# sauloal/pykmer

Hardware: AMD Instinct MI355X
Metric: bp/s k-mer counted (k=15, 1 GPU) (higher is better)
Workload: dtype u8

## Files before the change

### pykmer_amd/csrc/kmer_part.hip

```cpp
#include <cstddef>
#include "part_common.h"

namespace pk {

__global__ __launch_bounds__(1024) void k_sample2(const uint32_t *__restrict__ in, const uint32_t *__restrict__ bucket_base,
                                                  const uint32_t *__restrict__ bucket_end, PartPlan pl, uint32_t stride2,
                                                  uint32_t *__restrict__ tally, uint32_t *__restrict__ sampled_n,
                                                  const uint32_t *__restrict__ flags) {
    __shared__ uint32_t h[512];
    __shared__ uint32_t n_seen;
    if (flags[0]) return;
    const uint32_t b = blockIdx.x, lo = bucket_base[b], hi = bucket_end[b];
    if (threadIdx.x < 512) h[threadIdx.x] = 0;
    if (threadIdx.x == 0) n_seen = 0;
    __syncthreads();
    const uint32_t n_grp = (hi - lo + 255u) / 256u, n_sgrp = (n_grp + stride2 - 1u) / stride2;
    const uint32_t mask = pl.B2 - 1u, shift = pl.fb_bits, w = threadIdx.x >> 6, lane = threadIdx.x & 63u;
    uint32_t mine = 0;
    for (uint32_t s0 = 0; s0 < n_sgrp; s0 += 8u * 16u) {
        uint4 v[8];
        uint32_t n_ok[8];
#pragma unroll
        for (int u = 0; u < 8; u++) {
            const uint32_t sg = s0 + (uint32_t)u * 16u + w;
            const uint64_t i = (uint64_t)lo + (uint64_t)sg * stride2 * 256u + lane * 4u;
            n_ok[u] = (sg < n_sgrp && i < hi) ? (uint32_t)min((uint64_t)4, (uint64_t)hi - i) : 0u;
            v[u] = n_ok[u] ? *reinterpret_cast<const uint4 *>(in + i) : make_uint4(0, 0, 0, 0);
        }
#pragma unroll
        for (int u = 0; u < 8; u++) {
            const uint32_t r4[4] = {v[u].x, v[u].y, v[u].z, v[u].w};
#pragma unroll
            for (uint32_t e = 0; e < 4; e++)
                if (e < n_ok[u]) { atomicAdd(&h[(r4[e] >> shift) & mask], 1u); mine++; }
        }
    }
    for (int d = 32; d; d >>= 1) mine += __shfl_down(mine, d, 64);
    if ((threadIdx.x & 63) == 0 && mine) atomicAdd(&n_seen, mine);
    __syncthreads();
    if (threadIdx.x < pl.B2) tally[(uint64_t)b * pl.B2 + threadIdx.x] = h[threadIdx.x];
    if (threadIdx.x == 0) sampled_n[b] = n_seen;
}
__global__ __launch_bounds__(1024) void k_rooms2(const uint32_t *__restrict__ tally, const uint32_t *__restrict__ sampled_n,
                                                 const uint32_t *__restrict__ bucket_base, const uint32_t *__restrict__ bucket_end, PartPlan pl,
                                                 uint32_t stride2, uint32_t n_final, uint32_t *__restrict__ final_start,
                                                 uint32_t *__restrict__ cap2_end, uint32_t *__restrict__ block_tot, const uint32_t *__restrict__ flags) {
    __shared__ uint32_t wsum[16];
    if (flags[0]) return;
    const uint32_t i = blockIdx.x * 1024u + threadIdx.x;
    uint32_t room = 0;
    if (i < n_final) {
        const uint32_t b = i >> pl.b2, hcount = tally[i];
        if (stride2 == 1u) room = hcount;
        else {
            const uint32_t seen = sampled_n[b], n_b = bucket_end[b] - bucket_base[b];
            const unsigned long long est = seen ? (unsigned long long)((double)hcount * ((double)n_b / (double)seen)) + 1ull : 0ull;
            room = (uint32_t)(est + est / 4 + 4096u);
        }
        room = (room + 7u) & ~7u;
    }
    uint32_t inc = room;
    const int lane = threadIdx.x & 63, w = threadIdx.x >> 6;
#pragma unroll
    for (int d = 1; d < 64; d <<= 1) { const uint32_t o = __shfl_up(inc, d, 64); if (lane >= d) inc += o; }
    if (lane == 63) wsum[w] = inc;
    __syncthreads();
    uint32_t pre = 0, total = 0;
    for (int j = 0; j < 16; j++) { if (j < w) pre += wsum[j]; total += wsum[j]; }
    if (i < n_final) { final_start[i] = pre + inc - room; cap2_end[i] = room; }
    if (threadIdx.x == 0) block_tot[blockIdx.x] = total;
}
__global__ __launch_bounds__(1024) void k_bases2(uint32_t n_blocks, uint32_t n_final, PartPlan pl, uint32_t *__restrict__ block_tot,
                                                 uint32_t *__restrict__ final_start, uint32_t *__restrict__ flags) {
    __shared__ uint32_t wsum[16];
    if (flags[0]) return;
    const uint32_t v = threadIdx.x < n_blocks ? block_tot[threadIdx.x] : 0u;
    uint32_t inc = v;
    const int lane = threadIdx.x & 63, w = threadIdx.x >> 6;
#pragma unroll
    for (int d = 1; d < 64; d <<= 1) { const uint32_t o = __shfl_up(inc, d, 64); if (lane >= d) inc += o; }
    if (lane == 63) wsum[w] = inc;
    __syncthreads();
    uint32_t pre = 0, total = 0;
    for (int j = 0; j < 16; j++) { if (j < w) pre += wsum[j]; total += wsum[j]; }
    if (threadIdx.x < n_blocks) block_tot[threadIdx.x] = pre + inc - v;
    __shared__ unsigned long long total64;
    if (threadIdx.x == 0) total64 = 0ull;
    __syncthreads();
    unsigned long long mine = v;
    for (int d = 32; d; d >>= 1) mine += __shfl_down(mine, d, 64);
    if (lane == 0 && mine) atomicAdd(&total64, mine);
    __syncthreads();
    if (threadIdx.x == 0) {
        final_start[n_final] = total;
        if (total64 > pl.capacity2) flags[0] = 1u;
    }
}
__global__ __launch_bounds__(1024) void k_starts2(uint32_t n_final, const uint32_t *__restrict__ block_base, uint32_t *__restrict__ final_start,
                                                  uint32_t *__restrict__ cursor2, uint32_t *__restrict__ cap2_end, const uint32_t *__restrict__ flags) {
    if (flags[0]) return;
    const uint32_t i = blockIdx.x * 1024u + threadIdx.x;
    if (i >= n_final) return;
    const uint32_t a = block_base[blockIdx.x] + final_start[i];
    final_start[i] = a; cursor2[i] = a; cap2_end[i] = a + cap2_end[i];
}

template <int NT, int PER, bool REC24 = false>
__global__ __launch_bounds__(NT, 4) void k_scatter2(const uint32_t *__restrict__ in, const uint32_t *__restrict__ wg2_start,
                                                   const uint32_t *__restrict__ bucket_base, const uint32_t *__restrict__ bucket_end, PartPlan pl,
                                                   void *__restrict__ out, uint32_t *__restrict__ cursor, const uint32_t *__restrict__ cap_end,
                                                   uint32_t dump, uint32_t *__restrict__ flags) {
    extern __shared__ __attribute__((aligned(16))) uint8_t smem[];
    ScatterLds &L = *reinterpret_cast<ScatterLds *>(smem);
    if (flags[0]) return;
    const uint32_t B = pl.B2, shift = pl.fb_bits;
    const uint32_t low_mask = (1u << shift) - 1u;
    for (uint32_t i = threadIdx.x; i < 512; i += NT) { L.hist[i] = 0; L.run[i] = 0; }
    __syncthreads();
    typedef uint32_t Quad __attribute__((ext_vector_type(4)));
    typedef uint32_t Pair __attribute__((ext_vector_type(2)));
    const uint16_t *in_lo = reinterpret_cast<const uint16_t *>(in);
    const uint8_t *in_hi = reinterpret_cast<const uint8_t *>(in) + level1_hi_plane_offset(pl.capacity1);
    auto item = [&](uint32_t b, uint32_t lo, uint32_t hi) {
        auto fetch = [&](uint32_t win, Quad (&v)[PER / 4]) {
            const uint32_t v_hi = min(hi, win + (uint32_t)TILE);
#pragma unroll
            for (int j = 0; j < PER / 4; j++) {
                const uint32_t i = win + (threadIdx.x + j * NT) * 4u;
                v[j] = Quad{0u, 0u, 0u, 0u};
                if (i < v_hi) {
                    if (REC24) {
                        const Pair l = *reinterpret_cast<const Pair *>(in_lo + i);
                        v[j] = Quad{l.x, l.y, *reinterpret_cast<const uint32_t *>(in_hi + i), 0u};
                    } else v[j] = *reinterpret_cast<const Quad *>(in + i);
                }
            }
        };
        Quad nxt[PER / 4];
        auto settle = [&]() {
            __builtin_amdgcn_s_waitcnt(0x0F70);
#pragma unroll
            for (int j = 0; j < PER / 4; j++) asm volatile("" : "+v"(nxt[j]));
        };
        fetch(lo & ~3u, nxt);
        settle();
        for (uint32_t win = lo & ~3u; win < hi; win += TILE) {
            const uint32_t v_lo = max(lo, win), v_hi = min(hi, win + (uint32_t)TILE);
            const uint32_t n_tile = v_hi - v_lo;
            uint32_t r[PER];
#pragma unroll
            for (int j = 0; j < PER / 4; j++) {
                if (REC24) {
                    r[j * 4] = __builtin_amdgcn_perm(nxt[j].z, nxt[j].x, 0x0c040100u);
                    r[j * 4 + 1] = __builtin_amdgcn_perm(nxt[j].z, nxt[j].x, 0x0c050302u);
                    r[j * 4 + 2] = __builtin_amdgcn_perm(nxt[j].z, nxt[j].y, 0x0c060100u);
                    r[j * 4 + 3] = __builtin_amdgcn_perm(nxt[j].z, nxt[j].y, 0x0c070302u);
                } else { r[j * 4] = nxt[j].x; r[j * 4 + 1] = nxt[j].y; r[j * 4 + 2] = nxt[j].z; r[j * 4 + 3] = nxt[j].w; }
            }
            const bool full = v_lo == win && n_tile == (uint32_t)TILE;
            uint32_t okm = 0;
            if (!full) {
#pragma unroll
                for (int j = 0; j < PER / 4; j++) {
                    const uint32_t i = win + (threadIdx.x + j * NT) * 4u;
#pragma unroll
                    for (int e = 0; e < 4; e++) okm |= (i + e >= v_lo && i + e < v_hi) ? (1u << (j * 4 + e)) : 0u;
                }
            }
            if (win + TILE < hi) fetch(win + TILE, nxt);
            uint32_t *cl = cursor + (uint64_t)b * B;
            const uint32_t *ce = cap_end + (uint64_t)b * B;
            if (full) scatter_tile<uint32_t, false, NT, PER, 512, true, 8, REC24>(L, r, 0u, n_tile, shift, B, low_mask, true, out, settle, cl, ce, dump, flags);
            else scatter_tile<uint32_t, false, NT, PER, 512, false, 8, REC24>(L, r, okm, n_tile, shift, B, low_mask, true, out, settle, cl, ce, dump, flags);
        }
    };
    const uint32_t *pos = wg2_start;
    const uint32_t per = pl.B1 >> 3;
    const uint32_t o_lo = (blockIdx.x & 7u) * per, o_hi = o_lo + per, first = blockIdx.x >> 3, step = gridDim.x >> 3;
    const uint32_t w_end = pos[o_hi];
    for (uint32_t w = pos[o_lo] + first; w < w_end; w += step) {
        uint32_t a = o_lo, z = o_hi;
        while (z - a > 1) { const uint32_t m = (a + z) >> 1; if (pos[m] <= w) a = m; else z = m; }
        const uint32_t b = (a % per) * 8u + a / per;
        const uint64_t s = (uint64_t)bucket_base[b] + (uint64_t)(w - pos[a]) * pl.R2;
        const uint64_t e = min(s + pl.R2, (uint64_t)bucket_end[b]);
        item(b, (uint32_t)s, (uint32_t)e);
    }
}

constexpr uint32_t K6_PIECE = 65024;
constexpr int K6_BYTES_LDS = 65536 + 1024 + 128;

__device__ __forceinline__ int wave_sum_i32(int v) {
    v += __builtin_amdgcn_update_dpp(0, v, 0x128, 0xf, 0xf, false);
    v += __builtin_amdgcn_update_dpp(0, v, 0x124, 0xf, 0xf, false);
    v += __builtin_amdgcn_update_dpp(0, v, 0x122, 0xf, 0xf, false);
    v += __builtin_amdgcn_update_dpp(0, v, 0x121, 0xf, 0xf, false);
    return __builtin_amdgcn_readlane(v, 0) + __builtin_amdgcn_readlane(v, 16) + __builtin_amdgcn_readlane(v, 32) +
           __builtin_amdgcn_readlane(v, 48);
}

typedef unsigned short U16x2 __attribute__((ext_vector_type(2)));
__device__ __forceinline__ uint32_t clamp255_pair(uint32_t x) {
    const U16x2 lim = {255, 255};
    return __builtin_bit_cast(uint32_t, __builtin_elementwise_min(__builtin_bit_cast(U16x2, x), lim));
}
__device__ __forceinline__ uint32_t pack_low_bytes(uint32_t x0, uint32_t x1) {
    return __builtin_amdgcn_perm(x1, x0, 0x06040200u);
}

struct SliceTally {
    int d1 = 0, d2 = 0;
    __device__ __forceinline__ void add_dword(int *dh, uint32_t x, int sign) {
        uint32_t p0 = x & 0x01010101u, p1 = (x >> 1) & 0x01010101u;
        uint32_t rest = p0 & p1;
        const uint32_t high = x & 0xfcfcfcfcu;
        if (high) {
            const uint32_t big = (((high & 0x7f7f7f7fu) + 0x7f7f7f7fu) | high) & 0x80808080u;
            const uint32_t keep = ~(big >> 7);
            p0 &= keep; p1 &= keep;
            rest = (p0 & p1) | (big >> 7);
        }
        const int n1 = (int)__builtin_popcount(p0 & ~p1), n2 = (int)__builtin_popcount(p1 & ~p0);
        d1 += sign * n1; d2 += sign * n2;
        while (rest) {
            const int bit = __ffs(rest) - 1;
            atomicAdd(&dh[(x >> bit) & 0xffu], sign);
            rest &= rest - 1u;
        }
    }
};

template <int T, bool LEAN, bool NOREC = false>
__device__ __forceinline__ void bucket_count_body(const uint16_t *__restrict__ recs, const uint32_t *__restrict__ final_start,
                                                  const uint32_t *__restrict__ final_end, uint32_t fb_bits, uint32_t split_bits,
                                                  uint8_t *__restrict__ table8, uint32_t fresh, unsigned long long *__restrict__ hist_rep, uint8_t *smem,
                                                  int *dh, uint32_t wg) {
    uint32_t *cnt = reinterpret_cast<uint32_t *>(smem);
    const uint32_t fb = wg >> split_bits, part = wg & ((1u << split_bits) - 1u);
    const uint32_t start = final_start[fb], end = final_end ? final_end[fb] : final_start[fb + 1];
    const uint32_t part_bits = fb_bits - split_bits;
    const uint32_t n_addr = 1u << part_bits;
    uint8_t *slice = table8 + ((uint64_t)fb << fb_bits) + (uint64_t)part * n_addr;
    if (start == end) {
        if (fresh) {
            if (n_addr >= 16) for (uint32_t g = threadIdx.x; g < n_addr / 16; g += T) reinterpret_cast<uint4 *>(slice)[g] = make_uint4(0, 0, 0, 0);
            else for (uint32_t a = threadIdx.x; a < n_addr; a += T) slice[a] = 0;
        }
        return;
    }
    const uint32_t base = start & ~7u;
    const uint32_t i_first = base + threadIdx.x * 8;
    uint4 v_first = make_uint4(0, 0, 0, 0);
    if (i_first < min(base + K6_PIECE, end)) v_first = *reinterpret_cast<const uint4 *>(recs + i_first);
    const bool by_rec = NOREC ? false : (((end - start) >> split_bits) < n_addr / 4 || n_addr < 16);
    SliceTally tally;
    for (uint32_t i = threadIdx.x; i < 256; i += T) dh[i] = 0;
    if (fresh) {
        if (n_addr >= 8) for (uint32_t g = threadIdx.x; g < n_addr / 8; g += T) reinterpret_cast<uint4 *>(cnt)[g] = make_uint4(0, 0, 0, 0);
        else for (uint32_t a = threadIdx.x; a < max(n_addr / 2, 1u); a += T) cnt[a] = 0u;
    } else if (n_addr >= 16) {
        if (!by_rec) __syncthreads();
        for (uint32_t g = threadIdx.x; g < n_addr / 16; g += T) {
            uint4 v = reinterpret_cast<const uint4 *>(slice)[g];
            uint32_t w[4] = {v.x, v.y, v.z, v.w};
            if (!by_rec) {
#pragma unroll
                for (int q = 0; q < 4; q++) tally.add_dword(dh, w[q], -1);
            }
#pragma unroll
            for (int q = 0; q < 8; q++)
                cnt[g * 8 + q] = __builtin_amdgcn_perm(0u, w[q >> 1], (q & 1) ? 0x0c030c02u : 0x0c010c00u);
        }
    } else {
        for (uint32_t a = threadIdx.x; a < n_addr / 2; a += T) cnt[a] = slice[2 * a] | ((uint32_t)slice[2 * a + 1] << 16);
    }
    __syncthreads();
    auto bump = [&](uint32_t a, uint32_t n) {
        const uint32_t sh = 16u * (a & 1u);
        if (!by_rec) { atomicAdd(&cnt[a >> 1], n << sh); return; }
        int &d1 = tally.d1, &d2 = tally.d2;
        const uint32_t c = (atomicAdd(&cnt[a >> 1], n << sh) >> sh) & 0xffffu;
        const uint32_t oc = c > 255u ? 255u : c, nc = c + n > 255u ? 255u : c + n;
        if (oc == nc) return;
        if (nc == 1u) d1++;
        else if (nc == 2u && oc == 1u) { d2++; d1--; }
        else {
            atomicAdd(&dh[nc], 1);
            if (oc) atomicAdd(&dh[oc], -1);
        }
    };
    auto count8 = [&](const uint4 &v, uint32_t i) {
        const uint32_t w[4] = {v.x, v.y, v.z, v.w};
        if (LEAN && !by_rec) {
            const bool interior = i >= start && i + 8u <= end;
            uint8_t *cb = reinterpret_cast<uint8_t *>(cnt);
#pragma unroll
            for (int q = 0; q < 8; q++) {
                const uint32_t x = w[q >> 1];
                const uint32_t off = (q & 1) ? ((x >> 15) & 0x1fffcu) : ((x << 1) & 0x1fffcu);
                const uint32_t low = (q & 1) ? ((x >> 16) & 1u) : (x & 1u);
                uint32_t val = low * 0xffffu + 1u;
                if (!interior) val = (i + q >= start && i + q < end) ? val : 0u;
                __hip_atomic_fetch_add(reinterpret_cast<uint32_t *>(cb + off), val, __ATOMIC_RELAXED, __HIP_MEMORY_SCOPE_WORKGROUP);
            }
            return;
        }
        uint32_t pa = 0, pn = 0;
#pragma unroll
        for (int q = 0; q < 8; q++) {
            const uint32_t idx = i + q;
            const uint32_t full = (w[q >> 1] >> (16 * (q & 1))) & 0xffffu;
            const bool in = idx >= start && idx < end && (full >> part_bits) == part;
            const uint32_t a = full & (n_addr - 1u);
            if (in && pn && a == pa) pn++;
            else {
                if (pn) bump(pa, pn);
                pa = a; pn = in ? 1u : 0u;
            }
        }
        if (pn) bump(pa, pn);
    };
    auto count8_sparse = [&](const uint4 &v, uint32_t i) {
        const uint32_t w[4] = {v.x, v.y, v.z, v.w};
        uint32_t old[8];
        bool in[8];
        const bool interior = i >= start && i + 8u <= end;
#pragma unroll
        for (int q = 0; q < 8; q++) {
            const uint32_t idx = i + q;
            const uint32_t full = (w[q >> 1] >> (16 * (q & 1))) & 0xffffu;
            in[q] = (interior || (idx >= start && idx < end)) && (full >> part_bits) == part;
            const uint32_t a = full & (n_addr - 1u), sh = 16u * (a & 1u);
            old[q] = (atomicAdd(&cnt[a >> 1], in[q] ? (1u << sh) : 0u) >> sh) & 0xffffu;
        }
#pragma unroll
        for (int q = 0; q < 8; q++) {
            const uint32_t c = old[q];
            if (!in[q] || c >= 255u) continue;
            if (c == 0u) tally.d1++;
            else if (c == 1u) { tally.d2++; tally.d1--; }
            else { atomicAdd(&dh[c + 1u], 1); atomicAdd(&dh[c], -1); }
        }
    };
    constexpr int NIT = (K6_PIECE + T * 8 - 1) / (T * 8);
    if (end - base <= (uint32_t)T * 8u) {
        if (i_first < end) { if (by_rec) count8_sparse(v_first, i_first); else count8(v_first, i_first); }
        __syncthreads();
    } else {
        for (uint32_t p0 = base; p0 < end; p0 += K6_PIECE) {
            const uint32_t p1 = min(p0 + K6_PIECE, end);
            uint4 v[NIT];
#pragma unroll
            for (int it = 0; it < NIT; it++) {
                const uint32_t i = p0 + (threadIdx.x + it * T) * 8;
                v[it] = make_uint4(0, 0, 0, 0);
                if (i < p1) v[it] = (it == 0 && p0 == base) ? v_first : *reinterpret_cast<const uint4 *>(recs + i);
            }
#pragma unroll
            for (int it = 0; it < NIT; it++) {
                const uint32_t i = p0 + (threadIdx.x + it * T) * 8;
                if (i < p1) count8(v[it], i);
            }
            __syncthreads();
            if (p1 < end) {
                for (uint32_t a = threadIdx.x; a < max(n_addr / 2, 1u); a += T) {
                    cnt[a] = clamp255_pair(cnt[a]);
                }
                __syncthreads();
            }
        }
    }
    if (n_addr >= 16) {
        for (uint32_t g = threadIdx.x; g < n_addr / 16; g += T) {
            const uint4 c0 = reinterpret_cast<const uint4 *>(cnt)[g * 2], c1 = reinterpret_cast<const uint4 *>(cnt)[g * 2 + 1];
            const uint32_t o[4] = {pack_low_bytes(clamp255_pair(c0.x), clamp255_pair(c0.y)), pack_low_bytes(clamp255_pair(c0.z), clamp255_pair(c0.w)),
                                   pack_low_bytes(clamp255_pair(c1.x), clamp255_pair(c1.y)), pack_low_bytes(clamp255_pair(c1.z), clamp255_pair(c1.w))};
            if (!by_rec) {
#pragma unroll
                for (int q = 0; q < 4; q++) tally.add_dword(dh, o[q], 1);
            }
            reinterpret_cast<uint4 *>(slice)[g] = make_uint4(o[0], o[1], o[2], o[3]);
        }
    } else {
        for (uint32_t a = threadIdx.x; a < n_addr / 2; a += T) {
            uint32_t x = cnt[a], lo = x & 0xffffu, hi = x >> 16;
            slice[2 * a] = (uint8_t)(lo > 255u ? 255u : lo);
            slice[2 * a + 1] = (uint8_t)(hi > 255u ? 255u : hi);
        }
    }
    const int d1 = wave_sum_i32(tally.d1), d2 = wave_sum_i32(tally.d2);
    if ((threadIdx.x & 63) == 0) {
        if (d1) atomicAdd(&dh[1], d1);
        if (d2) atomicAdd(&dh[2], d2);
    }
    __syncthreads();
    for (uint32_t i = threadIdx.x; i < 256; i += T) {
        const int v = dh[i];
        if (v) atomicAdd(&hist_rep[(uint64_t)(blockIdx.x % HIST_REPLICAS) * 256 + i], (unsigned long long)(long long)v);
    }
}

template <int T>
__global__ __launch_bounds__(T) void k_bucket_count(const uint16_t *__restrict__ recs, const uint32_t *__restrict__ final_start,
                                                    const uint32_t *__restrict__ final_end, uint32_t fb_bits, uint32_t split_bits,
                                                    uint8_t *__restrict__ table8, uint32_t fresh, unsigned long long *__restrict__ hist_rep,
                                                    const uint32_t *__restrict__ flags) {
    extern __shared__ __attribute__((aligned(16))) uint8_t smem[];
    __shared__ int dh[256];
    if (flags[0]) return;
    bucket_count_body<T, true>(recs, final_start, final_end, fb_bits, split_bits, table8, fresh, hist_rep, smem, dh, blockIdx.x);
}
template <int T, bool FRESH>
__global__ __launch_bounds__(T) __attribute__((amdgpu_waves_per_eu(8, 8)))
void k_bucket_count_half_lean(const uint16_t *__restrict__ recs, const uint32_t *__restrict__ final_start, const uint32_t *__restrict__ final_end,
                              uint32_t fb_bits, uint32_t split_bits, uint8_t *__restrict__ table8, uint32_t fresh, unsigned long long *__restrict__ hist_rep,
                              const uint32_t *__restrict__ flags) {
    extern __shared__ __attribute__((aligned(16))) uint8_t smem[];
    __shared__ int dh[256];
    if (flags[0]) return;
    bucket_count_body<T, true, true>(recs, final_start, final_end, 15u, 0u, table8, FRESH ? 1u : 0u, hist_rep, smem, dh, blockIdx.x);
}

template <int T>
__global__ __launch_bounds__(T) __attribute__((amdgpu_waves_per_eu(8, 8)))
void k_bucket_count_bytes(const uint16_t *__restrict__ recs, const uint32_t *__restrict__ final_start, const uint32_t *__restrict__ final_end,
                          uint8_t *__restrict__ table8, uint32_t fresh, unsigned long long *__restrict__ hist_rep,
                          const uint32_t *__restrict__ flags) {
    extern __shared__ __attribute__((aligned(128))) uint8_t smem[];
    constexpr uint32_t N_ADDR = 65536u;
    int *dh = reinterpret_cast<int *>(smem + N_ADDR);
    uint32_t *wrap_flag = reinterpret_cast<uint32_t *>(smem + N_ADDR + 1024);
    if (flags[0]) return;
    const uint32_t fb = blockIdx.x;
    const uint32_t start = final_start[fb], end = final_end ? final_end[fb] : final_start[fb + 1];
    uint4 *slice = reinterpret_cast<uint4 *>(table8 + ((uint64_t)fb << 16));
    uint4 *img = reinterpret_cast<uint4 *>(smem);
    if (start == end) {
        if (fresh) for (uint32_t g = threadIdx.x; g < N_ADDR / 16; g += T) slice[g] = make_uint4(0, 0, 0, 0);
        return;
    }
    bool recount = end - start >= 16384u;
    int d1 = 0, d2 = 0;
    if (!recount) {
        const uint32_t base = start & ~7u;
        const uint32_t i_first = base + threadIdx.x * 8;
        uint4 v = make_uint4(0, 0, 0, 0);
        if (i_first < end) v = *reinterpret_cast<const uint4 *>(recs + i_first);
        for (uint32_t i = threadIdx.x; i < 256; i += T) dh[i] = 0;
        if (threadIdx.x == 0) *wrap_flag = 0u;
        if (fresh) { for (uint32_t g = threadIdx.x; g < N_ADDR / 16; g += T) img[g] = make_uint4(0, 0, 0, 0); }
        else { for (uint32_t g = threadIdx.x; g < N_ADDR / 16; g += T) img[g] = slice[g]; }
        __syncthreads();
        uint32_t *cnt = reinterpret_cast<uint32_t *>(smem);
        bool wrapped = false;
        for (uint32_t p0 = base; p0 < end; p0 += (uint32_t)T * 8u) {
            const uint32_t i = p0 + threadIdx.x * 8;
            if (i >= end) continue;
            if (p0 != base) v = *reinterpret_cast<const uint4 *>(recs + i);
            const uint32_t w[4] = {v.x, v.y, v.z, v.w};
            const bool interior = i >= start && i + 8u <= end;
            uint32_t old[8];
            bool in[8];
#pragma unroll
            for (int q = 0; q < 8; q++) {
                const uint32_t a = (w[q >> 1] >> (16 * (q & 1))) & 0xffffu, sh = 8u * (a & 3u);
                in[q] = interior || (i + q >= start && i + q < end);
                old[q] = (atomicAdd(&cnt[a >> 2], in[q] ? (1u << sh) : 0u) >> sh) & 0xffu;
            }
#pragma unroll
            for (int q = 0; q < 8; q++) {
                const uint32_t c = old[q];
                if (!in[q]) continue;
                if (c == 0u) d1++;
                else if (c == 1u) { d2++; d1--; }
                else if (c == 255u) wrapped = true;
                else { atomicAdd(&dh[c + 1u], 1); atomicAdd(&dh[c], -1); }
            }
        }
        if (wrapped) *wrap_flag = 1u;
        __syncthreads();
        recount = *wrap_flag != 0u;
        __syncthreads();
    }
    if (recount) {
        if (threadIdx.x == 0) atomicAdd(const_cast<uint32_t *>(&flags[1]), 1u);
        bucket_count_body<T, false>(recs, final_start, final_end, 16u, 1u, table8, fresh, hist_rep, smem, dh, 2u * fb);
        __syncthreads();
        bucket_count_body<T, false>(recs, final_start, final_end, 16u, 1u, table8, fresh, hist_rep, smem, dh, 2u * fb + 1u);
        return;
    }
    for (uint32_t g = threadIdx.x; g < N_ADDR / 16; g += T) slice[g] = img[g];
    d1 = wave_sum_i32(d1); d2 = wave_sum_i32(d2);
    if ((threadIdx.x & 63) == 0) {
        if (d1) atomicAdd(&dh[1], d1);
        if (d2) atomicAdd(&dh[2], d2);
    }
    __syncthreads();
    for (uint32_t i = threadIdx.x; i < 256; i += T) {
        const int x = dh[i];
        if (x) atomicAdd(&hist_rep[(uint64_t)(blockIdx.x % HIST_REPLICAS) * 256 + i], (unsigned long long)(long long)x);
    }
}

__device__ __forceinline__ void hist_reduce(unsigned long long *__restrict__ hist_rep, unsigned long long *__restrict__ hist) {
    if (threadIdx.x >= 256) return;
    unsigned long long acc = 0;
    for (uint32_t r = 0; r < HIST_REPLICAS; r++) {
        acc += hist_rep[(uint64_t)r * 256 + threadIdx.x];
        hist_rep[(uint64_t)r * 256 + threadIdx.x] = 0ull;
    }
    if (acc) atomicAdd(&hist[threadIdx.x], acc);
}

constexpr uint32_t AS_SLOTS = 4096, AS_WGS = 64;

__device__ __forceinline__ void table_sat_add(uint8_t *table8, uint64_t addr, uint32_t cnt, int *dh) {
    unsigned int *word = reinterpret_cast<unsigned int *>(table8 + (addr & ~3ull));
    const uint32_t sh = (uint32_t)(addr & 3ull) * 8u;
    unsigned int old = *word;
    while (true) {
        uint32_t b = (old >> sh) & 0xffu;
        uint32_t nb = b + cnt > 255u ? 255u : b + cnt;
        if (nb == b) return;
        unsigned int want = (old & ~(0xffu << sh)) | (nb << sh);
        unsigned int prev = atomicCAS(word, old, want);
        if (prev == old) {
            atomicAdd(&dh[nb], 1);
            if (b) atomicAdd(&dh[b], -1);
            return;
        }
        old = prev;
    }
}

__global__ __launch_bounds__(WG) void k_apply_side(const unsigned long long *__restrict__ side, const unsigned long long *__restrict__ side_n,
                                                   uint64_t side_cap, uint8_t *__restrict__ table8, unsigned long long *__restrict__ hist,
                                                   unsigned long long *__restrict__ hist_rep, const uint32_t *__restrict__ flags) {
    __shared__ unsigned long long key[AS_SLOTS];
    if (flags[0]) return;
    static_assert(WG >= 256, "one thread per histogram bin");
    if (blockIdx.x == 0) hist_reduce(hist_rep, hist);
    __shared__ uint32_t val[AS_SLOTS];
    __shared__ int dh[256];
    unsigned long long n = *side_n;
    if (n > side_cap) n = side_cap;
    const unsigned long long per = (n + gridDim.x - 1) / gridDim.x;
    const unsigned long long lo = per * blockIdx.x, hi = lo + per < n ? lo + per : n;
    if (lo >= hi) return;
    for (uint32_t i = threadIdx.x; i < AS_SLOTS; i += WG) { key[i] = 0ull; val[i] = 0u; }
    dh[threadIdx.x & 255u] = 0;
    __syncthreads();
    for (unsigned long long i = lo + threadIdx.x; i < hi; i += WG) {
        const unsigned long long e = side[i];
        const uint64_t addr = e >> SIDE_CNT_BITS;
        const uint32_t cnt = (uint32_t)(e & ((1ull << SIDE_CNT_BITS) - 1ull));
        const unsigned long long kk = addr + 1ull;
        uint32_t h = (uint32_t)((addr * 0x9E3779B97F4A7C15ull) >> 40) & (AS_SLOTS - 1u);
        bool done = false;
        for (uint32_t t = 0; t < 32 && !done; t++) {
            unsigned long long old = atomicCAS(&key[h], 0ull, kk);
            if (old == 0ull || old == kk) {
                uint32_t before = atomicAdd(&val[h], cnt);
                if (before + cnt < before) atomicExch(&val[h], 0xffffffffu);
                done = true;
            }
            h = (h + 1u) & (AS_SLOTS - 1u);
        }
        if (!done) table_sat_add(table8, addr, cnt > 255u ? 255u : cnt, dh);
    }
    __syncthreads();
    for (uint32_t i = threadIdx.x; i < AS_SLOTS; i += WG)
        if (key[i] != 0ull) table_sat_add(table8, key[i] - 1ull, val[i] > 255u ? 255u : val[i], dh);
    __syncthreads();
    if (threadIdx.x < 256 && dh[threadIdx.x]) atomicAdd(&hist[threadIdx.x], (unsigned long long)(long long)dh[threadIdx.x]);
}

PartPlan make_part_plan(uint32_t k, uint64_t n_bytes, uint32_t slice_bits, uint32_t slice_index) {
    PartPlan pl;
    pl.k = k;
    pl.slice_bits = slice_bits;
    pl.slice_index = slice_index;
    pl.addr_bits = 2 * k - slice_bits;
    pl.fb_bits = pl.addr_bits < 16 ? pl.addr_bits : 16;
    if (k <= 15 && pl.addr_bits >= 24 && n_bytes >= (((uint64_t)1 << pl.addr_bits) >> 3)) pl.fb_bits = 15;
    const uint32_t bucket_bits = pl.addr_bits - pl.fb_bits;
    const uint32_t one_level_max = k <= 15 ? 7u : 9u;
    pl.b1 = bucket_bits <= one_level_max ? bucket_bits : (bucket_bits + 1) / 2;
    if (pl.b1 > one_level_max) pl.b1 = one_level_max;
    pl.b2 = bucket_bits - pl.b1;
    pl.B1 = 1u << pl.b1;
    pl.B2 = 1u << pl.b2;
    pl.n_chunks = (uint32_t)((n_bytes + CHUNK - 1) / CHUNK);
    pl.n_wg0 = pl.n_chunks < 1024u ? pl.n_chunks : 1024u;
    if (pl.n_wg0 == 0) pl.n_wg0 = 1;
    pl.G = (pl.n_chunks + pl.n_wg0 - 1) / pl.n_wg0;
    if (pl.G == 0) pl.G = 1;
    const uint32_t wg1 = 4096u;
    pl.n_wg1 = pl.n_chunks < wg1 ? pl.n_chunks : wg1;
    if (pl.n_wg1 == 0) pl.n_wg1 = 1;
    pl.G1 = (pl.n_chunks + pl.n_wg1 - 1) / pl.n_wg1;
    if (pl.G1 == 0) pl.G1 = 1;
    pl.R2 = 4u * TILE;
    pl.sample_stride = pl.n_chunks >= 1024u ? 16u : 1u;
    const uint64_t nfb = (uint64_t)pl.B1 * pl.B2;
    pl.n_tally = (pl.b2 && nfb <= 32768 && pl.addr_bits <= 30) ? (uint32_t)nfb : pl.B1;
    pl.sample2 = (pl.b2 && pl.n_tally == pl.B1 && nfb <= 262144 && pl.B1 >= 8u) ? 1u : 0u;
    const uint64_t est1 = (uint64_t)pl.n_chunks * TILE + pl.B1, est2 = (uint64_t)pl.n_chunks * TILE + nfb;
    pl.capacity1 = est1 + est1 / 8 + (uint64_t)pl.B1 * 4100;
    pl.capacity2 = pl.sample2 ? est2 + est2 / 4 + nfb * 4104 : est2 + est2 / 8 + nfb * 2056;
    return pl;
}

size_t part_workspace_bytes(const PartPlan &pl, uint64_t n_bytes, PartWorkspace *lay) {
    auto up = [](size_t x) { return (x + 255) & ~(size_t)255; };
    const uint64_t nfb = (uint64_t)pl.B1 * pl.B2;
    size_t o = 0;
    lay->codes = o; o += up((size_t)pl.n_chunks * SLOT_CODE_WORDS * 4);
    lay->restarts = o; o += up((size_t)pl.n_chunks * SLOT_RST_WORDS * 4);
    lay->n_bases = o; o += up((size_t)pl.n_chunks * 4);
    lay->tally_rows = o; o += up((size_t)COUNT_WGS * pl.n_tally * 4);
    lay->tally_tot = o; o += up(pl.sample2 ? (size_t)nfb * 4 + (size_t)(pl.B1 + 1024) * 4 : (size_t)pl.n_tally * 4);
    lay->bucket_base = o; o += up((size_t)(pl.B1 + 1) * 4);
    lay->bucket_end = o; o += up((size_t)(pl.B1 + 1) * 4);
    lay->cursor1 = o; o += up((size_t)(pl.B1 + 1) * 4);
    lay->cap_end = o; o += up((size_t)(pl.B1 + 1) * 4);
    lay->wg2_start = o; o += up((size_t)(pl.B1 + 1) * 4);
    lay->final_start = o; o += up((size_t)(nfb + 1) * 4);
    lay->cursor2 = o; o += up((size_t)(nfb + 1) * 4);
    lay->cap2_end = o; o += up((size_t)(nfb + 1) * 4);
    lay->out1 = o; o += !pl.b2 ? up((size_t)(pl.capacity1 + TILE + 64) * 2)
                     : pl.k <= 15 ? level1_hi_plane_offset(pl.capacity1) + up((size_t)(pl.capacity1 + TILE + 64))
                                  : up((size_t)(pl.capacity1 + TILE + 64) * 4);
    lay->out2 = o; o += up(!pl.b2 ? 256 : (size_t)(pl.capacity2 + TILE + 64) * 2);
    lay->side_cap = n_bytes + 16;
    lay->side = o; o += up((size_t)lay->side_cap * 8);
    lay->side_n = o; o += 256;
    return o;
}

void part_set_attributes() {
    fuse_set_attributes();
    hipFuncSetAttribute((const void *)k_scatter2<512, 32>, hipFuncAttributeMaxDynamicSharedMemorySize, (int)SCATTER_LDS_NARROW);
    hipFuncSetAttribute((const void *)k_scatter2<512, 32, true>, hipFuncAttributeMaxDynamicSharedMemorySize, (int)SCATTER_LDS_NARROW);
    hipFuncSetAttribute((const void *)k_bucket_count<1024>, hipFuncAttributeMaxDynamicSharedMemorySize, 128 * 1024);
    hipFuncSetAttribute((const void *)k_bucket_count_half_lean<1024, true>, hipFuncAttributeMaxDynamicSharedMemorySize, 128 * 1024);
    hipFuncSetAttribute((const void *)k_bucket_count_half_lean<1024, false>, hipFuncAttributeMaxDynamicSharedMemorySize, 128 * 1024);
    hipFuncSetAttribute((const void *)k_bucket_count_bytes<1024>, hipFuncAttributeMaxDynamicSharedMemorySize, K6_BYTES_LDS);
}

extern "C" int pk_diag_occupancy(int which) {
    int n = -1;
    hipError_t e = hipErrorInvalidValue;
    if (which == 0) e = hipOccupancyMaxActiveBlocksPerMultiprocessor(&n, (const void *)k_bucket_count<1024>, 1024, 128 * 1024);
    if (which == 1) e = hipOccupancyMaxActiveBlocksPerMultiprocessor(&n, (const void *)k_bucket_count_bytes<1024>, 1024, K6_BYTES_LDS);
    if (which == 2) e = hipOccupancyMaxActiveBlocksPerMultiprocessor(&n, (const void *)k_bucket_count_half_lean<1024, true>, 1024, 65536);
    if (which == 3) e = hipOccupancyMaxActiveBlocksPerMultiprocessor(&n, (const void *)k_scatter2<512, 32>, 512, SCATTER_LDS_NARROW);
    return e == hipSuccess ? n : -(int)e;
}

int launch_partitioned(const L2 *st2, uint64_t n_bytes, const PartPlan &pl, uint32_t stride, uint8_t *ws, const PartWorkspace &lay, uint8_t *table8,
                       hipStream_t s, hipEvent_t ev_sort_begin, hipEvent_t ev_sort_end, hipEvent_t ev_part_end, bool fresh,
                       unsigned long long *hist, unsigned long long *bucket_hist, bool armed) {
    const uint32_t *codes = (const uint32_t *)(ws + lay.codes), *restarts = (const uint32_t *)(ws + lay.restarts);
    const uint32_t *n_bases = (const uint32_t *)(ws + lay.n_bases);
    uint32_t *tally_rows = (uint32_t *)(ws + lay.tally_rows), *tally_tot = (uint32_t *)(ws + lay.tally_tot);
    uint32_t *bucket_base = (uint32_t *)(ws + lay.bucket_base), *bucket_end = (uint32_t *)(ws + lay.bucket_end);
    uint32_t *cursor1 = (uint32_t *)(ws + lay.cursor1), *cap_end = (uint32_t *)(ws + lay.cap_end);
    uint32_t *wg2_start = (uint32_t *)(ws + lay.wg2_start), *final_start = (uint32_t *)(ws + lay.final_start);
    uint32_t *cursor2 = (uint32_t *)(ws + lay.cursor2), *cap2_end = (uint32_t *)(ws + lay.cap2_end);
    void *out1 = ws + lay.out1, *out2 = ws + lay.out2;
    unsigned long long *side = (unsigned long long *)(ws + lay.side), *side_n = (unsigned long long *)(ws + lay.side_n);
    uint32_t *flags = (uint32_t *)(side_n + 1);
    const uint32_t nfb = pl.B1 * pl.B2;
    const bool laid_out2 = pl.n_tally > pl.B1 || pl.sample2;
    if (pl.B1 > (pl.k <= 15 ? 128u : 512u) || pl.B2 > 512u || pl.fb_bits > 16u) return -3;
    if (pl.b2 && !laid_out2) return -3;
    if (pl.k <= 15 && pl.b2 && pl.addr_bits - pl.b1 > 24u) return -3;
    if (!armed && hipMemsetAsync(side_n, 0, PART_FLAG_WORDS * 4, s) != hipSuccess) return -2;
    launch_provision(codes, restarts, n_bases, st2, pl, stride, tally_rows, tally_tot, bucket_base, cursor1, cap_end, final_start, cursor2, cap2_end,
                     flags, s);
    if (ev_sort_begin) hipEventRecord(ev_sort_begin, s);
    launch_walk_sort(codes, restarts, n_bases, st2, pl, out1, cursor1, cap_end, flags, bucket_base, bucket_end, wg2_start, side, side_n, lay.side_cap, s);
    if (ev_sort_end) hipEventRecord(ev_sort_end, s);
    const uint16_t *final_recs = (const uint16_t *)out1;
    const uint32_t *k6_start = bucket_base, *k6_end = bucket_end;
    if (pl.sample2) {
        const uint32_t stride2 = stride == 1u ? 1u : 16u, n_blocks = (nfb + 1023u) / 1024u;
        uint32_t *sampled_n = tally_tot + nfb, *block_tot = sampled_n + pl.B1;
        hipLaunchKernelGGL(k_sample2, dim3(pl.B1), dim3(1024), 0, s, (const uint32_t *)out1, (const uint32_t *)bucket_base, (const uint32_t *)bucket_end,
                           pl, stride2, tally_tot, sampled_n, (const uint32_t *)flags);
        hipLaunchKernelGGL(k_rooms2, dim3(n_blocks), dim3(1024), 0, s, (const uint32_t *)tally_tot, (const uint32_t *)sampled_n,
                           (const uint32_t *)bucket_base, (const uint32_t *)bucket_end, pl, stride2, nfb, final_start, cap2_end, block_tot,
                           (const uint32_t *)flags);
        hipLaunchKernelGGL(k_bases2, dim3(1), dim3(1024), 0, s, n_blocks, nfb, pl, block_tot, final_start, flags);
        hipLaunchKernelGGL(k_starts2, dim3(n_blocks), dim3(1024), 0, s, nfb, (const uint32_t *)block_tot, final_start, cursor2, cap2_end,
                           (const uint32_t *)flags);
    }
    if (pl.b2) {
        const uint32_t grid2 = 4096u;
        if (pl.k <= 15)
            hipLaunchKernelGGL((k_scatter2<512, 32, true>), dim3(grid2), dim3(512), SCATTER_LDS_NARROW, s, (const uint32_t *)out1, wg2_start,
                               bucket_base, bucket_end, pl, out2, cursor2, (const uint32_t *)cap2_end, (uint32_t)pl.capacity2, flags);
        else
            hipLaunchKernelGGL((k_scatter2<512, 32>), dim3(grid2), dim3(512), SCATTER_LDS_NARROW, s, (const uint32_t *)out1, wg2_start,
                               bucket_base, bucket_end, pl, out2, cursor2, (const uint32_t *)cap2_end, (uint32_t)pl.capacity2, flags);
        final_recs = (const uint16_t *)out2; k6_start = final_start; k6_end = cursor2;
    }
    if (ev_part_end) hipEventRecord(ev_part_end, s);
    const bool sparse = pl.fb_bits == 16 && n_bytes / nfb < 8192u;
    const uint32_t split = sparse ? 1u : 0u;
    const size_t part_addrs = (size_t)1 << (pl.fb_bits - split);
    const size_t lds6 = part_addrs * 2 < 64 ? 64 : part_addrs * 2;
    const uint32_t n_rows6 = (uint32_t)(nfb << split);
    if (split > 1u) return -3;
    if (pl.fb_bits == 15 && fresh)
        hipLaunchKernelGGL((k_bucket_count_half_lean<1024, true>), dim3(n_rows6), dim3(1024), lds6, s, final_recs, k6_start, k6_end, pl.fb_bits, split, table8,
                           fresh ? 1u : 0u, bucket_hist, (const uint32_t *)flags);
    else if (pl.fb_bits == 15)
        hipLaunchKernelGGL((k_bucket_count_half_lean<1024, false>), dim3(n_rows6), dim3(1024), lds6, s, final_recs, k6_start, k6_end, pl.fb_bits, split, table8,
                           fresh ? 1u : 0u, bucket_hist, (const uint32_t *)flags);
    else if (split)
        hipLaunchKernelGGL(k_bucket_count_bytes<1024>, dim3(nfb), dim3(1024), K6_BYTES_LDS, s, final_recs, k6_start, k6_end, table8, fresh ? 1u : 0u, bucket_hist,
                           (const uint32_t *)flags);
    else
        hipLaunchKernelGGL(k_bucket_count<1024>, dim3(n_rows6), dim3(1024), lds6, s, final_recs, k6_start, k6_end, pl.fb_bits, split, table8,
                           fresh ? 1u : 0u, bucket_hist, (const uint32_t *)flags);
    hipLaunchKernelGGL(k_apply_side, dim3(AS_WGS), dim3(WG), 0, s, side, side_n, lay.side_cap, table8, hist, bucket_hist, (const uint32_t *)flags);
    return hipGetLastError() == hipSuccess ? 0 : -2;
}

}
```

### pykmer_amd/csrc/pk_kernels.h

```cpp
#pragma once
#include <hip/hip_runtime.h>
#include <stdint.h>
#include "fasta_fsm.h"

namespace pk {

struct DevRec {
    uint64_t name_off;
    uint64_t name_end;
    uint64_t seq_len;
    uint64_t n_valid;
};

struct Carry {
    L2 l2;
    L1 l1;
    uint32_t pad;
    uint64_t n_recs;
    uint64_t total_bp;
    uint64_t num_kmers;
};

void launch_chunk_l1(const uint8_t *fasta, uint64_t n, L1 *chunk_l1, uint32_t n_chunks, hipStream_t s);
void launch_scan_l1(const L1 *in, uint32_t n_chunks, Carry *carry, L1 *out, L1 *tile_ws, uint32_t *zero_words, uint32_t n_zero, hipStream_t s);
void launch_chunk_l2(const uint8_t *fasta, uint64_t n, const L1 *st1, L2 *chunk_l2, LaneState *lane_state, PiecePack *packs, uint32_t *chunk_odd, uint32_t n_chunks,
                     uint32_t k, hipStream_t s);
void launch_scan_l2(const L2 *in, uint32_t n_chunks, Carry *carry, L2 *out, L2 *tile_ws, uint32_t k, hipStream_t s);
void launch_hist8(const uint8_t *table8, uint64_t n, unsigned long long *hist, hipStream_t s);

constexpr uint32_t SLOT_CODE_WORDS = 1024;
constexpr uint32_t SLOT_RST_WORDS = 512;
void launch_squeeze(const uint8_t *fasta, uint64_t n, uint64_t stream_off, const LaneState *lane_state, const PiecePack *packs, const L2 *st2,
                    const uint32_t *chunk_odd, uint32_t k, uint32_t n_chunks, uint32_t n_wg, uint32_t chunks_per_wg, uint32_t *codes, uint32_t *restarts, uint32_t *n_bases,
                    DevRec *recs, uint64_t recs_cap, Carry *carry, uint32_t *flags, hipStream_t s);

struct PartPlan {
    uint32_t k, addr_bits;
    uint32_t slice_bits, slice_index;
    uint32_t fb_bits;
    uint32_t b1, b2, B1, B2;
    uint32_t n_chunks;
    uint32_t n_wg0, G;
    uint32_t n_wg1, G1;
    uint64_t R2;
    uint32_t sample_stride;
    uint32_t n_tally;
    uint32_t sample2;
    uint64_t capacity1;
    uint64_t capacity2;
};
constexpr uint32_t COUNT_WGS = 256;
struct PartWorkspace {
    size_t codes, restarts, n_bases, tally_rows, tally_tot, bucket_base, bucket_end, cursor1, cap_end, wg2_start, final_start, cursor2, cap2_end,
        out1, out2, side, side_n;
    uint64_t side_cap;
};
PartPlan make_part_plan(uint32_t k, uint64_t n_bytes, uint32_t slice_bits, uint32_t slice_index);
size_t part_workspace_bytes(const PartPlan &pl, uint64_t n_bytes, PartWorkspace *lay);
void part_set_attributes();
void fuse_set_attributes();
void launch_provision(const uint32_t *codes, const uint32_t *restarts, const uint32_t *n_bases, const L2 *st2, const PartPlan &pl,
                      uint32_t stride, uint32_t *tally_rows, uint32_t *tally_tot, uint32_t *bucket_base, uint32_t *cursor1,
                      uint32_t *cap_end, uint32_t *final_start, uint32_t *cursor2, uint32_t *cap2_end, uint32_t *flags, hipStream_t s);
void launch_walk_sort(const uint32_t *codes, const uint32_t *restarts, const uint32_t *n_bases, const L2 *st2, const PartPlan &pl, void *out1,
                      uint32_t *cursor1, const uint32_t *cap_end, uint32_t *flags, const uint32_t *bucket_base, uint32_t *bucket_end,
                      uint32_t *wg2_start, unsigned long long *side, unsigned long long *side_n, uint64_t side_cap, hipStream_t s);
int launch_partitioned(const L2 *st2, uint64_t n_bytes, const PartPlan &pl, uint32_t stride, uint8_t *ws, const PartWorkspace &lay, uint8_t *table8,
                       hipStream_t s, hipEvent_t ev_sort_begin, hipEvent_t ev_sort_end, hipEvent_t ev_part_end, bool fresh,
                       unsigned long long *hist, unsigned long long *hist_replicas, bool armed);
constexpr uint32_t HIST_REPLICAS = 64;
constexpr uint32_t PART_FLAG_WORDS = 6;

int launch_gram(const uint8_t *const *dev_tables, int N, uint64_t n_slice, int min_count, int max_count,
                unsigned long long *dev_pair, bool zero_first, hipStream_t s);

int gram_windows_per_pass(int N);
int launch_gram_windows(const uint8_t *const *dev_tables, int N, uint64_t n_slice, const int *min_counts, const int *max_counts,
                        const int *out_index, int W, unsigned long long *dev_pair, hipStream_t s);

int spectrum_groups(int N);
int launch_spectrum(const void *const *dev_tables, int N, uint64_t n_slice, unsigned long long *dev_accum, const uint8_t **host_gtab,
                    const uint8_t **dev_gtab, hipStream_t s);

uint64_t occgram_scratch_bytes(int N, uint64_t n_slice);
int launch_occgram(const void *const *dev_tables, int N, uint64_t n_slice, unsigned long long *dev_accum, const uint8_t **dev_ptrs,
                   uint8_t *occ_scratch, hipStream_t s);

}
```

Measured before the change: 217.6 billion.

## Count final buckets with 8-bit LDS image and wrap-detect recount fallback

Replaces the 16-bit-per-address half-lean bucket counter with a 512-thread kernel that keeps a 32 KB byte-per-address image in LDS and increments packed bytes with workgroup-scope atomics. Each block checks whether the image sum matches the record count. If a byte counter wrapped, the bucket goes onto a recount list handled by a second 1024-thread kernel. Oversized buckets are found up front and split across dedicated workgroups. The aim is to halve LDS use for higher occupancy and cheaper atomics, at the cost of an extra launch, an extra recount pass for overflowing buckets, and more complexity.

```diff
diff --git a/pykmer_amd/csrc/kmer_part.hip b/pykmer_amd/csrc/kmer_part.hip
--- a/pykmer_amd/csrc/kmer_part.hip
+++ b/pykmer_amd/csrc/kmer_part.hip
@@ -231,7 +231,7 @@
     }
 };
 
-template <int T, bool LEAN, bool NOREC = false>
+template <int T, bool LEAN, bool NOREC = false, uint32_t PIECE = K6_PIECE>
 __device__ __forceinline__ void bucket_count_body(const uint16_t *__restrict__ recs, const uint32_t *__restrict__ final_start,
                                                   const uint32_t *__restrict__ final_end, uint32_t fb_bits, uint32_t split_bits,
                                                   uint8_t *__restrict__ table8, uint32_t fresh, unsigned long long *__restrict__ hist_rep, uint8_t *smem,
@@ -252,7 +252,7 @@
     const uint32_t base = start & ~7u;
     const uint32_t i_first = base + threadIdx.x * 8;
     uint4 v_first = make_uint4(0, 0, 0, 0);
-    if (i_first < min(base + K6_PIECE, end)) v_first = *reinterpret_cast<const uint4 *>(recs + i_first);
+    if (i_first < min(base + PIECE, end)) v_first = *reinterpret_cast<const uint4 *>(recs + i_first);
     const bool by_rec = NOREC ? false : (((end - start) >> split_bits) < n_addr / 4 || n_addr < 16);
     SliceTally tally;
     for (uint32_t i = threadIdx.x; i < 256; i += T) dh[i] = 0;
@@ -343,13 +343,13 @@
             else { atomicAdd(&dh[c + 1u], 1); atomicAdd(&dh[c], -1); }
         }
     };
-    constexpr int NIT = (K6_PIECE + T * 8 - 1) / (T * 8);
+    constexpr int NIT = (PIECE + T * 8 - 1) / (T * 8);
     if (end - base <= (uint32_t)T * 8u) {
         if (i_first < end) { if (by_rec) count8_sparse(v_first, i_first); else count8(v_first, i_first); }
         __syncthreads();
     } else {
-        for (uint32_t p0 = base; p0 < end; p0 += K6_PIECE) {
-            const uint32_t p1 = min(p0 + K6_PIECE, end);
+        for (uint32_t p0 = base; p0 < end; p0 += PIECE) {
+            const uint32_t p1 = min(p0 + PIECE, end);
             uint4 v[NIT];
 #pragma unroll
             for (int it = 0; it < NIT; it++) {
@@ -411,16 +411,173 @@
     if (flags[0]) return;
     bucket_count_body<T, true>(recs, final_start, final_end, fb_bits, split_bits, table8, fresh, hist_rep, smem, dh, blockIdx.x);
 }
+constexpr uint32_t IMG_ADDR = 32768;
+constexpr uint32_t IMG_OUTSIZED = 65536;
+constexpr int K6_IMG_LDS = IMG_ADDR + 1024 + 64;
+
+struct ImageTally {
+    int d1 = 0, d2 = 0, d3 = 0, sum = 0;
+    __device__ __forceinline__ void add_dword(int *dh, uint32_t x, int sign) {
+        if (sign > 0) sum = (int)__builtin_amdgcn_udot4(x, 0x01010101u, (uint32_t)sum, false);
+        else sum -= (int)__builtin_amdgcn_udot4(x, 0x01010101u, 0u, false);
+        const uint32_t h = x >> 1, p0 = x & 0x01010101u, p1 = h & 0x01010101u;
+        const uint32_t big = (((h & 0x7e7e7e7eu) + 0x7e7e7e7eu) >> 7) & 0x01010101u;
+        const uint32_t small = ~big;
+        d1 += sign * (int)__builtin_popcount(p0 & ~p1 & small);
+        d2 += sign * (int)__builtin_popcount(p1 & ~p0 & small);
+        d3 += sign * (int)__builtin_popcount(p0 & p1 & small);
+#pragma unroll
+        for (int j = 0; j < 4; j++)
+            if ((big >> (8 * j)) & 1u) atomicAdd(&dh[(x >> (8 * j)) & 0xffu], sign);
+    }
+};
+
+template <int T>
+__device__ uint32_t find_outsized(const uint32_t *__restrict__ final_start, const uint32_t *__restrict__ final_end, uint32_t nfb, uint32_t want,
+                                  uint32_t *lds) {
+    constexpr uint32_t NW = T / 64;
+    const uint32_t lane = threadIdx.x & 63u, w = threadIdx.x >> 6;
+    const uint32_t per = (nfb + NW - 1u) / NW, lo = min(w * per, nfb), hi = min(lo + per, nfb);
+    auto big = [&](uint32_t b) { return b < hi && (final_end ? final_end[b] : final_start[b + 1]) - final_start[b] >= IMG_OUTSIZED; };
+    uint32_t n = 0;
+    for (uint32_t b0 = lo; b0 < hi; b0 += 64u) n += (uint32_t)__popcll(__ballot(big(b0 + lane)));
+    if (lane == 0) lds[w] = n;
+    if (threadIdx.x == 0) lds[NW] = ~0u;
+    __syncthreads();
+    uint32_t pre = 0;
+    for (uint32_t j = 0; j < w; j++) pre += lds[j];
+    if (want >= pre && want < pre + n) {
+        uint32_t r = want - pre;
+        for (uint32_t b0 = lo; b0 < hi; b0 += 64u) {
+            unsigned long long m = __ballot(big(b0 + lane));
+            const uint32_t c = (uint32_t)__popcll(m);
+            if (r < c) {
+                for (uint32_t q = 0; q < r; q++) m &= m - 1ull;
+                if (lane == 0) lds[NW] = b0 + (uint32_t)__ffsll((long long)m) - 1u;
+                break;
+            }
+            r -= c;
+        }
+    }
+    __syncthreads();
+    return lds[NW];
+}
+
+constexpr uint32_t OUT_SLOTS = 64, OUT_SPLIT = 3, OUT_PARTS = 1u << OUT_SPLIT, OUT_WGS = OUT_SLOTS * OUT_PARTS;
+
 template <int T, bool FRESH>
 __global__ __launch_bounds__(T) __attribute__((amdgpu_waves_per_eu(8, 8)))
-void k_bucket_count_half_lean(const uint16_t *__restrict__ recs, const uint32_t *__restrict__ final_start, const uint32_t *__restrict__ final_end,
-                              uint32_t fb_bits, uint32_t split_bits, uint8_t *__restrict__ table8, uint32_t fresh, unsigned long long *__restrict__ hist_rep,
-                              const uint32_t *__restrict__ flags) {
+void k_bucket_count_image(const uint16_t *__restrict__ recs, const uint32_t *__restrict__ final_start, const uint32_t *__restrict__ final_end,
+                          uint32_t nfb, uint8_t *__restrict__ table8, unsigned long long *__restrict__ hist_rep, uint32_t *__restrict__ recount_list,
+                          const uint32_t *__restrict__ flags) {
+    extern __shared__ __attribute__((aligned(128))) uint8_t smem[];
+    constexpr int NW = T / 64, NG = (int)IMG_ADDR / 16 / T;
+    uint32_t *img = reinterpret_cast<uint32_t *>(smem);
+    int *dh = reinterpret_cast<int *>(smem + IMG_ADDR);
+    int *wsum = reinterpret_cast<int *>(smem + IMG_ADDR + 1024);
+    if (flags[0]) return;
+    if (blockIdx.x < OUT_WGS) {
+        const uint32_t ob = find_outsized<T>(final_start, final_end, nfb, blockIdx.x / OUT_PARTS, reinterpret_cast<uint32_t *>(wsum));
+        if (ob != ~0u)
+            bucket_count_body<T, false, true, (uint32_t)T * 64u>(recs, final_start, final_end, 15u, OUT_SPLIT, table8, FRESH ? 1u : 0u, hist_rep, smem, dh,
+                                                                 ob * OUT_PARTS + blockIdx.x % OUT_PARTS);
+        return;
+    }
+    const uint32_t fb = blockIdx.x - OUT_WGS;
+    const uint32_t start = final_start[fb], end = final_end ? final_end[fb] : final_start[fb + 1];
+    uint4 *slice = reinterpret_cast<uint4 *>(table8 + ((uint64_t)fb << 15));
+    if (start == end) {
+        if (FRESH) for (uint32_t g = threadIdx.x; g < IMG_ADDR / 16; g += T) slice[g] = make_uint4(0, 0, 0, 0);
+        return;
+    }
+    bool recount = end - start >= IMG_OUTSIZED;
+    if (recount) {
+        const uint32_t last = find_outsized<T>(final_start, final_end, nfb, OUT_SLOTS - 1u, reinterpret_cast<uint32_t *>(wsum));
+        if (last == ~0u || last >= fb) return;
+    } else {
+        const uint32_t a0 = (start + 7u) & ~7u, a1 = end & ~7u;
+        uint4 v = make_uint4(0, 0, 0, 0);
+        if (a0 + threadIdx.x * 8u < a1) v = *reinterpret_cast<const uint4 *>(recs + a0 + threadIdx.x * 8u);
+        for (uint32_t i = threadIdx.x; i < 256; i += T) dh[i] = 0;
+        ImageTally tally;
+        if (FRESH) {
+            for (uint32_t g = threadIdx.x; g < IMG_ADDR / 16; g += T) reinterpret_cast<uint4 *>(img)[g] = make_uint4(0, 0, 0, 0);
+        } else {
+            __syncthreads();
+#pragma unroll 1
+            for (int u = 0; u < NG; u++) {
+                const uint32_t g = threadIdx.x + (uint32_t)u * T;
+                const uint4 x = slice[g];
+                reinterpret_cast<uint4 *>(img)[g] = x;
+                tally.add_dword(dh, x.x, -1); tally.add_dword(dh, x.y, -1);
+                tally.add_dword(dh, x.z, -1); tally.add_dword(dh, x.w, -1);
+            }
+        }
+        __syncthreads();
+        auto add = [&](uint32_t a) {
+            __hip_atomic_fetch_add(img + ((a >> 2) & (IMG_ADDR / 4 - 1u)), 1u << ((a << 3) & 24u), __ATOMIC_RELAXED, __HIP_MEMORY_SCOPE_WORKGROUP);
+        };
+        if (threadIdx.x < 16u) {
+            const uint32_t i = threadIdx.x < 8u ? start + threadIdx.x : max(a0, a1) + threadIdx.x - 8u;
+            if (i < (threadIdx.x < 8u ? min(a0, end) : end)) add(recs[i]);
+        }
+        for (uint32_t p = a0; p < a1; p += (uint32_t)T * 8u) {
+            const uint32_t i = p + threadIdx.x * 8u;
+            if (i >= a1) break;
+            uint4 nx = make_uint4(0, 0, 0, 0);
+            if (i + (uint32_t)T * 8u < a1) nx = *reinterpret_cast<const uint4 *>(recs + i + (uint32_t)T * 8u);
+            const uint32_t w[4] = {v.x, v.y, v.z, v.w};
+#pragma unroll
+            for (int q = 0; q < 4; q++) { add(w[q]); add(w[q] >> 16); }
+            v = nx;
+        }
+        __syncthreads();
+        uint4 o[NG];
+#pragma unroll
+        for (int u = 0; u < NG; u++) {
+            o[u] = reinterpret_cast<const uint4 *>(img)[threadIdx.x + (uint32_t)u * T];
+            tally.add_dword(dh, o[u].x, 1); tally.add_dword(dh, o[u].y, 1);
+            tally.add_dword(dh, o[u].z, 1); tally.add_dword(dh, o[u].w, 1);
+        }
+        const int s = wave_sum_i32(tally.sum);
+        if ((threadIdx.x & 63u) == 0) wsum[threadIdx.x >> 6] = s;
+        __syncthreads();
+        int total = 0;
+#pragma unroll
+        for (int j = 0; j < NW; j++) total += wsum[j];
+        recount = total != (int)(end - start);
+        if (!recount) {
+#pragma unroll
+            for (int u = 0; u < NG; u++) slice[threadIdx.x + (uint32_t)u * T] = o[u];
+            const int d1 = wave_sum_i32(tally.d1), d2 = wave_sum_i32(tally.d2), d3 = wave_sum_i32(tally.d3);
+            if ((threadIdx.x & 63u) == 0) {
+                if (d1) atomicAdd(&dh[1], d1);
+                if (d2) atomicAdd(&dh[2], d2);
+                if (d3) atomicAdd(&dh[3], d3);
+            }
+            __syncthreads();
+            for (uint32_t i = threadIdx.x; i < 256; i += T) {
+                const int x = dh[i];
+                if (x) atomicAdd(&hist_rep[(uint64_t)(blockIdx.x % HIST_REPLICAS) * 256 + i], (unsigned long long)(long long)x);
+            }
+            return;
+        }
+    }
+    if (threadIdx.x == 0) recount_list[atomicAdd(const_cast<uint32_t *>(&flags[1]), 1u)] = fb;
+}
+
+template <bool FRESH>
+__global__ __launch_bounds__(1024) __attribute__((amdgpu_waves_per_eu(8, 8)))
+void k_bucket_recount(const uint16_t *__restrict__ recs, const uint32_t *__restrict__ final_start, const uint32_t *__restrict__ final_end,
+                      uint8_t *__restrict__ table8, unsigned long long *__restrict__ hist_rep, const uint32_t *__restrict__ recount_list,
+                      const uint32_t *__restrict__ flags) {
     extern __shared__ __attribute__((aligned(16))) uint8_t smem[];
     __shared__ int dh[256];
     if (flags[0]) return;
-    bucket_count_body<T, true, true>(recs, final_start, final_end, 15u, 0u, table8, FRESH ? 1u : 0u, hist_rep, smem, dh, blockIdx.x);
-}
+    if (blockIdx.x >= flags[1]) return;
+    bucket_count_body<1024, false, true>(recs, final_start, final_end, 15u, 0u, table8, FRESH ? 1u : 0u, hist_rep, smem, dh, recount_list[blockIdx.x]);
+}
+
 
 template <int T>
 __global__ __launch_bounds__(T) __attribute__((amdgpu_waves_per_eu(8, 8)))
@@ -636,6 +793,7 @@
     lay->side_cap = n_bytes + 16;
     lay->side = o; o += up((size_t)lay->side_cap * 8);
     lay->side_n = o; o += 256;
+    lay->recount = o; o += up((size_t)nfb * 4);
     return o;
 }
 
@@ -644,8 +802,10 @@
     hipFuncSetAttribute((const void *)k_scatter2<512, 32>, hipFuncAttributeMaxDynamicSharedMemorySize, (int)SCATTER_LDS_NARROW);
     hipFuncSetAttribute((const void *)k_scatter2<512, 32, true>, hipFuncAttributeMaxDynamicSharedMemorySize, (int)SCATTER_LDS_NARROW);
     hipFuncSetAttribute((const void *)k_bucket_count<1024>, hipFuncAttributeMaxDynamicSharedMemorySize, 128 * 1024);
-    hipFuncSetAttribute((const void *)k_bucket_count_half_lean<1024, true>, hipFuncAttributeMaxDynamicSharedMemorySize, 128 * 1024);
-    hipFuncSetAttribute((const void *)k_bucket_count_half_lean<1024, false>, hipFuncAttributeMaxDynamicSharedMemorySize, 128 * 1024);
+    hipFuncSetAttribute((const void *)k_bucket_count_image<512, true>, hipFuncAttributeMaxDynamicSharedMemorySize, K6_IMG_LDS);
+    hipFuncSetAttribute((const void *)k_bucket_count_image<512, false>, hipFuncAttributeMaxDynamicSharedMemorySize, K6_IMG_LDS);
+    hipFuncSetAttribute((const void *)k_bucket_recount<true>, hipFuncAttributeMaxDynamicSharedMemorySize, 65536);
+    hipFuncSetAttribute((const void *)k_bucket_recount<false>, hipFuncAttributeMaxDynamicSharedMemorySize, 65536);
     hipFuncSetAttribute((const void *)k_bucket_count_bytes<1024>, hipFuncAttributeMaxDynamicSharedMemorySize, K6_BYTES_LDS);
 }
 
@@ -654,7 +814,8 @@
     hipError_t e = hipErrorInvalidValue;
     if (which == 0) e = hipOccupancyMaxActiveBlocksPerMultiprocessor(&n, (const void *)k_bucket_count<1024>, 1024, 128 * 1024);
     if (which == 1) e = hipOccupancyMaxActiveBlocksPerMultiprocessor(&n, (const void *)k_bucket_count_bytes<1024>, 1024, K6_BYTES_LDS);
-    if (which == 2) e = hipOccupancyMaxActiveBlocksPerMultiprocessor(&n, (const void *)k_bucket_count_half_lean<1024, true>, 1024, 65536);
+    if (which == 2) e = hipOccupancyMaxActiveBlocksPerMultiprocessor(&n, (const void *)k_bucket_count_image<512, true>, 512, K6_IMG_LDS);
+    if (which == 4) e = hipOccupancyMaxActiveBlocksPerMultiprocessor(&n, (const void *)k_bucket_recount<true>, 1024, 65536);
     if (which == 3) e = hipOccupancyMaxActiveBlocksPerMultiprocessor(&n, (const void *)k_scatter2<512, 32>, 512, SCATTER_LDS_NARROW);
     return e == hipSuccess ? n : -(int)e;
 }
@@ -672,6 +833,7 @@
     void *out1 = ws + lay.out1, *out2 = ws + lay.out2;
     unsigned long long *side = (unsigned long long *)(ws + lay.side), *side_n = (unsigned long long *)(ws + lay.side_n);
     uint32_t *flags = (uint32_t *)(side_n + 1);
+    uint32_t *recount = (uint32_t *)(ws + lay.recount);
     const uint32_t nfb = pl.B1 * pl.B2;
     const bool laid_out2 = pl.n_tally > pl.B1 || pl.sample2;
     if (pl.B1 > (pl.k <= 15 ? 128u : 512u) || pl.B2 > 512u || pl.fb_bits > 16u) return -3;
@@ -714,12 +876,20 @@
     const size_t lds6 = part_addrs * 2 < 64 ? 64 : part_addrs * 2;
     const uint32_t n_rows6 = (uint32_t)(nfb << split);
     if (split > 1u) return -3;
-    if (pl.fb_bits == 15 && fresh)
-        hipLaunchKernelGGL((k_bucket_count_half_lean<1024, true>), dim3(n_rows6), dim3(1024), lds6, s, final_recs, k6_start, k6_end, pl.fb_bits, split, table8,
-                           fresh ? 1u : 0u, bucket_hist, (const uint32_t *)flags);
-    else if (pl.fb_bits == 15)
-        hipLaunchKernelGGL((k_bucket_count_half_lean<1024, false>), dim3(n_rows6), dim3(1024), lds6, s, final_recs, k6_start, k6_end, pl.fb_bits, split, table8,
-                           fresh ? 1u : 0u, bucket_hist, (const uint32_t *)flags);
+    if (pl.fb_bits == 15) {
+        if (fresh)
+            hipLaunchKernelGGL((k_bucket_count_image<512, true>), dim3(OUT_WGS + nfb), dim3(512), K6_IMG_LDS, s, final_recs, k6_start, k6_end, nfb, table8,
+                               bucket_hist, recount, (const uint32_t *)flags);
+        else
+            hipLaunchKernelGGL((k_bucket_count_image<512, false>), dim3(OUT_WGS + nfb), dim3(512), K6_IMG_LDS, s, final_recs, k6_start, k6_end, nfb, table8,
+                               bucket_hist, recount, (const uint32_t *)flags);
+        if (fresh)
+            hipLaunchKernelGGL(k_bucket_recount<true>, dim3(nfb), dim3(1024), 65536, s, final_recs, k6_start, k6_end, table8, bucket_hist,
+                               (const uint32_t *)recount, (const uint32_t *)flags);
+        else
+            hipLaunchKernelGGL(k_bucket_recount<false>, dim3(nfb), dim3(1024), 65536, s, final_recs, k6_start, k6_end, table8, bucket_hist,
+                               (const uint32_t *)recount, (const uint32_t *)flags);
+    }
     else if (split)
         hipLaunchKernelGGL(k_bucket_count_bytes<1024>, dim3(nfb), dim3(1024), K6_BYTES_LDS, s, final_recs, k6_start, k6_end, table8, fresh ? 1u : 0u, bucket_hist,
                            (const uint32_t *)flags);
diff --git a/pykmer_amd/csrc/pk_kernels.h b/pykmer_amd/csrc/pk_kernels.h
--- a/pykmer_amd/csrc/pk_kernels.h
+++ b/pykmer_amd/csrc/pk_kernels.h
@@ -52,7 +52,7 @@
 constexpr uint32_t COUNT_WGS = 256;
 struct PartWorkspace {
     size_t codes, restarts, n_bases, tally_rows, tally_tot, bucket_base, bucket_end, cursor1, cap_end, wg2_start, final_start, cursor2, cap2_end,
-        out1, out2, side, side_n;
+        out1, out2, side, side_n, recount;
     uint64_t side_cap;
 };
 PartPlan make_part_plan(uint32_t k, uint64_t n_bytes, uint32_t slice_bits, uint32_t slice_index);
```

New measurement: 218.2 billion (median of 6 runs). No clear change (+0.3%).
